# quadjr/aframe-gaussian-splatting

Hardware: AMD Instinct MI355X
Metric: frames/sec @1920x1080 (sort+project+bin+blend per frame, 1M-splat train.splat-shaped scene) (higher is better)
Workload: dtype f32

## Files before the change

aframe-gaussian-splatting_amd/csrc/gs_render.hip:

```cpp
#include "gs_internal.h"
#include "gs_sh.h"

namespace {

#define GS_DPP_ADD(V, CTRL, ROWS) (V) += (uint32_t)__builtin_amdgcn_update_dpp(0, (int)(V), (CTRL), (ROWS), 0xF, false)
__device__ __forceinline__ uint32_t row16_sum(uint32_t v)
{
#ifdef GS_DEBUG_DPP_MAX
    const uint32_t v0_ = v;
#endif
    GS_DPP_ADD(v, 0xB1, 0xF);
    GS_DPP_ADD(v, 0x4E, 0xF);
    GS_DPP_ADD(v, 0x141, 0xF);
    GS_DPP_ADD(v, 0x140, 0xF);
#ifdef GS_DEBUG_DPP_MAX
    { uint32_t c = v0_; for (int m = 8; m >= 1; m >>= 1) c += __shfl_xor(c, m, 16); if (c != v) __builtin_trap(); }
#endif
    return v;
}
__device__ __forceinline__ uint32_t wave_sum(uint32_t v)
{
#ifdef GS_DEBUG_DPP_MAX
    uint32_t c_ = v; for (int m = 32; m >= 1; m >>= 1) c_ += __shfl_xor(c_, m, 64);
#endif
// ... 538 lines not shown
#pragma unroll
        for (uint32_t k = 0; k < 4; k++) {
            s_rrun[4u * l + k] = er; s_rpair[4u * l + k] = ep; if (ITEMS) s_item[4u * l + k] = ei;
            er += rt[k].x; ep += rt[k].y; ei += ni[k];
        }
        if (l == 63) { s_rrun[GS_BLOCK] = er; s_rpair[GS_BLOCK] = ep; if (ITEMS) s_item[GS_BLOCK] = ei; *s_total = sp64; }
    }
    __syncthreads();
    return *s_total;
}

template <int ROUND>
__device__ __forceinline__ void k_row_scan_body(uint32_t *__restrict__ row_cnt, uint2 *__restrict__ row_tot, const GsControl *ctl,
                                                uint32_t near_count, uint32_t rc_stride, uint32_t tiles_y, uint32_t *__restrict__ mask,
                                                uint32_t mask_words)
{
    __shared__ uint32_t s_w[4];
    __shared__ unsigned long long s_p[4];
    uint32_t j_lo, j_hi;
    round_range<ROUND>(ctl, near_count, j_lo, j_hi);
    const uint32_t nch = (j_hi - j_lo + GS_BLOCK - 1) / GS_BLOCK;
    const int lane = threadIdx.x & 63, w = threadIdx.x >> 6;
    const uint32_t per = (nch + GS_BLOCK - 1) / GS_BLOCK;
    const uint32_t lo = min(threadIdx.x * per, nch), hi = min(lo + per, nch);
    for (uint32_t row = blockIdx.x; row < tiles_y; row += gridDim.x) {
        if (ROUND == 0) for (uint32_t i = threadIdx.x; i < mask_words; i += GS_BLOCK) mask[row * mask_words + i] = 0u;
        uint32_t *__restrict__ rc = row_cnt + (size_t)row * rc_stride;
        uint32_t sr = 0;
        unsigned long long sp = 0;
        for (uint32_t c = lo; c < hi; c++) { const uint32_t v = rc[c]; sr += v & 0x1FFu; sp += v >> 9; }
        uint32_t total;
        uint32_t run = block_exscan(sr, s_w, lane, w, total);
        const unsigned long long tp = block_sum64(sp, s_p, lane, w);
        for (uint32_t c = lo; c < hi; c++) { const uint32_t v = rc[c]; rc[c] = run; run += v & 0x1FFu; }
        if (threadIdx.x == 0) row_tot[row] = make_uint2(total, tp > 0xFFFFFFFFull ? 0xFFFFFFFFu : (uint32_t)tp);
    }
}

template <int ROUND>
__global__ __launch_bounds__(GS_BLOCK) void k_row_scan(uint32_t *__restrict__ row_cnt, uint2 *__restrict__ row_tot, const GsControl *ctl,
                                                       uint32_t near_count, uint32_t rc_stride, uint32_t tiles_y, uint32_t *__restrict__ mask,
                                                       uint32_t mask_words)
{
    k_row_scan_body<ROUND>(row_cnt, row_tot, ctl, near_count, rc_stride, tiles_y, mask, mask_words);
}

template <int ROUND>
__device__ __forceinline__ void round_books(GsControl *ctl, unsigned long long I, uint32_t runs, uint32_t j_lo, uint32_t j_hi, uint32_t near_count,
                                            const uint32_t *__restrict__ part_vis, uint32_t nparts, int last_round, uint32_t pair_cap)
{
    __shared__ uint32_t s_vis;
    const uint32_t tid = threadIdx.x;
    const int lane = threadIdx.x & 63;
    if (tid == 0) s_vis = 0;
    __syncthreads();
    uint32_t v = 0;
    if (j_hi > j_lo) for (uint32_t i = tid; i < nparts; i += GS_BLOCK) v += part_vis[i];
#pragma unroll
    for (int m = 32; m >= 1; m >>= 1) v += __shfl_xor(v, m, 64);
    if (lane == 0 && v) atomicAdd(&s_vis, v);
    __syncthreads();
    if (tid == 0) {
        const uint32_t total = I > 0xFFFFFFFFull ? 0xFFFFFFFFu : (uint32_t)I;
        ctl->vis_total = 0; ctl->n_emit_extra = 0;
        ctl->n_runs = (ROUND == 0 ? 0u : ctl->n_runs) + runs;
        if (ROUND == 0) { ctl->n_visible = 0; ctl->n_pairs_frame = 0; ctl->want_frame = 0; }
        else { ctl->unsat_round0 = ctl->unsat_count; if (ctl->unsat_count) ctl->unsat_events += 1; }
        ctl->j_lo = j_lo; ctl->j_hi = j_hi;
        ctl->scan_total = total;
        ctl->want_frame = (ctl->want_frame + total < total) ? 0xFFFFFFFFu : ctl->want_frame + total;
        if (ctl->want_frame > ctl->max_total) ctl->max_total = ctl->want_frame;
        if (total > pair_cap) { ctl->pair_overflow = 1; ctl->overflow_sticky = 1; ctl->n_pairs = 0; }
        else if (ROUND == 0) { ctl->pair_overflow = 0; ctl->n_pairs = total; }
        else ctl->n_pairs = ctl->pair_overflow ? 0u : total;
        ctl->n_visible += s_vis; ctl->n_pairs_frame += ctl->n_pairs;
        if (ROUND == 0 && near_count != 0xFFFFFFFFu) ctl->unsat_count = 0;
        if (last_round) {
            ctl->acc_frames += 1; ctl->acc_sorted += ctl->n_kept; ctl->acc_visible += ctl->n_visible; ctl->acc_pairs += ctl->n_pairs_frame;
        }
    }
    __syncthreads();
}

template <int ROUND>
__device__ __forceinline__ void k_emit_runs_body(const gsm::Projected *__restrict__ proj, const uint2 *__restrict__ rect,
                                                 const uint32_t *__restrict__ tile_count, const uint32_t *__restrict__ row_cnt,
                                                 const uint2 *__restrict__ row_tot, const GsFrameUniforms &u,
                                                 uint32_t *__restrict__ run_geom, uint32_t *__restrict__ run_ref,
                                                 const uint32_t *__restrict__ mask, GsControl *ctl, uint32_t pair_cap, uint2 *__restrict__ row_runs,
                                                 const uint32_t *__restrict__ part_vis, uint32_t nparts, int last_round)
{
    __shared__ float s_rec[GS_BLOCK][6];
    __shared__ uint32_t s_rows[GS_BLOCK], s_t[GS_BLOCK];
    __shared__ unsigned long long s_m[GS_BLOCK][4];
    __shared__ uint32_t s_rowrun[GS_BLOCK + 1], s_rowpair[GS_BLOCK + 1], s_base[GS_BLOCK];
    __shared__ uint32_t s_nbig, s_nmid;
    __shared__ unsigned long long s_p[4];
    const uint32_t tid = threadIdx.x;
    const int lane = threadIdx.x & 63, w = threadIdx.x >> 6;
    const uint32_t tiles_y = (uint32_t)u.tiles_y;
    const unsigned long long I = row_prefixes<false>(row_tot, tiles_y, s_rowrun, s_rowpair, nullptr, s_p);
    uint32_t j_lo, j_hi;
    round_range<ROUND>(ctl, u.near_count, j_lo, j_hi);
    const bool overflow = I > pair_cap || (ROUND == 1 && ctl->pair_overflow);
    if (blockIdx.x == 0) {
        round_books<ROUND>(ctl, I, s_rowrun[GS_BLOCK], j_lo, j_hi, u.near_count, part_vis, nparts, last_round, pair_cap);
        if (ROUND == 0 && tid < tiles_y) row_runs[tid] = make_uint2(s_rowrun[tid], overflow ? 0u : s_rowrun[tid + 1] - s_rowrun[tid]);
    }
    if (overflow) return;
    const uint32_t nchunks = (j_hi - j_lo + GS_BLOCK - 1) / GS_BLOCK;
    for (uint32_t c = blockIdx.x; c < nchunks; c += gridDim.x) {
        s_m[tid][0] = 0ull; s_m[tid][1] = 0ull; s_m[tid][2] = 0ull; s_m[tid][3] = 0ull;
        if (tid == 0) { s_nbig = 0; s_nmid = 0; }
        if (tid < tiles_y) s_base[tid] = s_rowrun[tid] + row_cnt[(size_t)tid * u.rc_stride + c];
        __syncthreads();
        const uint32_t j = j_lo + c * GS_BLOCK + tid;
        const uint32_t cnt = j < j_hi ? tile_count[j] : 0u;
        bool own = false;
        uint32_t ty0 = 0, ty1 = 0;
        gsm::Projected p;
        p.cx = p.cy = p.ax = p.ay = p.bx = p.by = 0.0f;
        uint32_t own_runs = 0, own_present = 0;
        if (cnt) {
            const uint2 rc = rect[j];
            if (rc.x & (1u << 14)) {
                own = true;
                ty0 = rc.x >> 16; ty1 = ty0 + ((rc.x >> 15) & 1u);
                own_runs = rc.y; own_present = (rc.x >> 12) & 3u;
            } else {
                const float4 *src = reinterpret_cast<const float4 *>(proj + j);
                const float4 ra = src[0]; const float2 rb = *reinterpret_cast<const float2 *>(src + 1);
                p.cx = ra.x; p.cy = ra.y; p.ax = ra.z; p.ay = ra.w; p.bx = rb.x; p.by = rb.y;
                ty0 = rc.x >> 16; ty1 = rc.y >> 16;
                const uint32_t q = (ty1 - ty0 >= 16) ? (GS_BLOCK - 1u - atomicAdd(&s_nbig, 1u)) : atomicAdd(&s_nmid, 1u);
                s_rec[q][0] = p.cx; s_rec[q][1] = p.cy; s_rec[q][2] = p.ax; s_rec[q][3] = p.ay; s_rec[q][4] = p.bx; s_rec[q][5] = p.by;
                s_rows[q] = ty0 | (ty1 << 16); s_t[q] = tid;
            }
        }
        __syncthreads();
        const uint32_t nmid = s_nmid, nbig = s_nbig;
#define GS_RUN_ONE(PP, EE, T, TY, FN) do { uint32_t a_, n_;                                                                       \
            gsm::splat_tile_row(PP, EE, (int)(TY), u.H, u.x0, u.x1b, a_, n_);                                                     \
            if (n_ && (ROUND == 0 || mask_count(mask + (TY) * u.mask_words, a_, n_))) { FN((T), (TY), a_, n_); } } while (0)
#define GS_RUN_PASS(FN) do {                                                                                                      \
            if (own) {                                                                                                            \
                for (uint32_t ty = ty0; ty <= ty1; ty++) if ((own_present >> (ty - ty0)) & 1u) {                                  \
                    const uint32_t r_ = own_runs >> (16u * (ty - ty0)), a_ = r_ & 0xFFu, n_ = ((r_ >> 8) & 0xFFu) + 1u;           \
                    if (ROUND == 0 || mask_count(mask + ty * u.mask_words, a_, n_)) { FN(tid, ty, a_, n_); } } }                  \
            for (uint32_t mi = (uint32_t)w * 4u + ((uint32_t)lane >> 4); mi < nmid; mi += 16u) {                                  \
                gsm::Projected q;                                                                                                 \
                q.cx = s_rec[mi][0]; q.cy = s_rec[mi][1]; q.ax = s_rec[mi][2]; q.ay = s_rec[mi][3]; q.bx = s_rec[mi][4]; q.by = s_rec[mi][5]; \
                gsm::EllipseRows e; gsm::ellipse_rows_setup(q, e);                                                                \
                const uint32_t ty = (s_rows[mi] & 0xFFFFu) + ((uint32_t)lane & 15u);                                              \
                if (ty <= (s_rows[mi] >> 16)) GS_RUN_ONE(q, e, s_t[mi], ty, FN); }                                                \
            for (uint32_t bq = (uint32_t)w; bq < nbig; bq += 4u) {                                                                \
                const uint32_t bi = GS_BLOCK - 1u - bq;                                                                           \
                gsm::Projected q;                                                                                                 \
                q.cx = s_rec[bi][0]; q.cy = s_rec[bi][1]; q.ax = s_rec[bi][2]; q.ay = s_rec[bi][3]; q.bx = s_rec[bi][4]; q.by = s_rec[bi][5]; \
                gsm::EllipseRows e; gsm::ellipse_rows_setup(q, e);                                                                \
                for (uint32_t ty = (s_rows[bi] & 0xFFFFu) + (uint32_t)lane; ty <= (s_rows[bi] >> 16); ty += 64u) GS_RUN_ONE(q, e, s_t[bi], ty, FN); } \
        } while (0)
#define GS_RUN_MARK(T, TY, A, N) atomicOr(&s_m[TY][(T) >> 6], 1ull << ((T) & 63u))
        GS_RUN_PASS(GS_RUN_MARK);
        __syncthreads();
#define GS_RUN_WRITE(T, TY, A, N) do { const uint32_t wq_ = (T) >> 6;                                                             \
            uint32_t rank_ = (uint32_t)__popcll(s_m[TY][wq_] & ((1ull << ((T) & 63u)) - 1ull));                                   \
            for (uint32_t k_ = 0; k_ < wq_; k_++) rank_ += (uint32_t)__popcll(s_m[TY][k_]);                                       \
            const uint32_t slot_ = s_base[TY] + rank_;                                                                            \
            run_geom[slot_] = (A) | ((N) << 16); run_ref[slot_] = j_lo + c * GS_BLOCK + (T); } while (0)
        GS_RUN_PASS(GS_RUN_WRITE);
#undef GS_RUN_WRITE
#undef GS_RUN_MARK
#undef GS_RUN_PASS
#undef GS_RUN_ONE
        __syncthreads();
    }
}

template <int ROUND>
__global__ __launch_bounds__(GS_BLOCK) void k_emit_runs(const gsm::Projected *__restrict__ proj, const uint2 *__restrict__ rect,
                                                        const uint32_t *__restrict__ tile_count, const uint32_t *__restrict__ row_cnt,
                                                        const uint2 *__restrict__ row_tot, GsFrameUniforms u,
                                                        uint32_t *__restrict__ run_geom, uint32_t *__restrict__ run_ref,
                                                        const uint32_t *__restrict__ mask, GsControl *ctl, uint32_t pair_cap, uint2 *__restrict__ row_runs,
                                                        const uint32_t *__restrict__ part_vis, uint32_t nparts, int last_round)
{
    k_emit_runs_body<ROUND>(proj, rect, tile_count, row_cnt, row_tot, u, run_geom, run_ref, mask, ctl, pair_cap, row_runs, part_vis, nparts, last_round);
}

template <int ROUND>
__device__ __forceinline__ void k_seg_count_body(const uint32_t *__restrict__ run_geom, const uint2 *__restrict__ row_tot, int *__restrict__ seg_diff,
                                                 const GsFrameUniforms &u, const GsControl *ctl, uint32_t pair_cap)
{
    __shared__ uint32_t s_rrun[GS_BLOCK + 1], s_rpair[GS_BLOCK + 1], s_item[GS_BLOCK + 1];
    __shared__ int s_d[GS_BLOCK + 1];
    __shared__ unsigned long long s_p[4];
    const uint32_t tid = threadIdx.x, tiles_y = (uint32_t)u.tiles_y;
    const unsigned long long I = row_prefixes<true>(row_tot, tiles_y, s_rrun, s_rpair, s_item, s_p);
    if (I > pair_cap || (ROUND == 1 && ctl->pair_overflow)) return;
    const uint32_t NI = s_item[GS_BLOCK];
    for (uint32_t item = blockIdx.x; item < NI; item += gridDim.x) {
        uint32_t row = 0;
#pragma unroll
        for (uint32_t step = GS_BLOCK / 2; step; step >>= 1) { const uint32_t t = row + step; if (t < tiles_y && s_item[t] <= item) row = t; }
        const uint32_t seg = item - s_item[row];
        const uint32_t rb = s_rrun[row], nr = s_rrun[row + 1] - rb;
        const uint32_t S = list_seg_len(nr), s0 = seg * S, s1 = min(nr, s0 + S);
        s_d[tid] = 0;
        if (tid == 0) s_d[GS_BLOCK] = 0;
        __syncthreads();
        for (uint32_t i0 = s0; i0 < s1; i0 += GS_LIST_LOADS * GS_BLOCK) {
            uint32_t g[GS_LIST_LOADS];
#pragma unroll
            for (uint32_t k = 0; k < GS_LIST_LOADS; k++) { const uint32_t i = i0 + k * GS_BLOCK + tid; g[k] = i < s1 ? run_geom[rb + i] : 0u; }
#pragma unroll
            for (uint32_t k = 0; k < GS_LIST_LOADS; k++) {
                const uint32_t i = i0 + k * GS_BLOCK + tid;
                if (i < s1) { const uint32_t t0 = g[k] & 0xFFFFu; atomicAdd(&s_d[t0], 1); atomicSub(&s_d[t0 + (g[k] >> 16)], 1); }
            }
        }
        __syncthreads();
        seg_diff[(size_t)item * GS_BLOCK + tid] = s_d[tid];
        __syncthreads();
    }
}

template <int ROUND>
__global__ __launch_bounds__(GS_BLOCK) void k_seg_count(const uint32_t *__restrict__ run_geom, const uint2 *__restrict__ row_tot, int *__restrict__ seg_diff,
                                                        GsFrameUniforms u, const GsControl *ctl, uint32_t pair_cap)
{
    k_seg_count_body<ROUND>(run_geom, row_tot, seg_diff, u, ctl, pair_cap);
}

__device__ __forceinline__ unsigned long long wave_incl_scan_u64(unsigned long long v, int lane)
{
#pragma unroll
    for (int d = 1; d < 64; d <<= 1) {
        const unsigned long long t = ((unsigned long long)__shfl_up((uint32_t)(v >> 32), d, 64) << 32) | __shfl_up((uint32_t)v, d, 64);
        if (lane >= d) v += t;
    }
    return v;
}

template <int ROUND, bool SEGC>
__device__ __forceinline__ void k_lists_body(const uint32_t *__restrict__ run_geom, const uint32_t *__restrict__ run_ref,
                                             const uint2 *__restrict__ row_tot, const int *__restrict__ seg_diff, uint32_t *__restrict__ lists, uint2 *__restrict__ tile_range,
                                             const GsFrameUniforms &u, const uint32_t *__restrict__ mask, const GsControl *ctl, uint32_t pair_cap)
{
    __shared__ uint32_t s_rrun[GS_BLOCK + 1], s_rpair[GS_BLOCK + 1], s_item[GS_BLOCK + 1];
    __shared__ unsigned long long s_d[GS_BLOCK + 1];
    __shared__ __attribute__((aligned(16))) unsigned long long s_m[GS_BLOCK][4];
    __shared__ uint32_t s_r[GS_BLOCK];
    __shared__ uint32_t s_off[GS_BLOCK], s_on[GS_BLOCK];
    __shared__ uint32_t s_w[4];
    __shared__ unsigned long long s_p[4];
    const uint32_t tid = threadIdx.x;
    const int lane = threadIdx.x & 63, w = threadIdx.x >> 6;
    const uint32_t tiles_x = (uint32_t)u.tiles_x, tiles_y = (uint32_t)u.tiles_y;
    const unsigned long long I = row_prefixes<true>(row_tot, tiles_y, s_rrun, s_rpair, s_item, s_p);
    const uint32_t NI = s_item[GS_BLOCK];
    const bool overflow = I > pair_cap || (ROUND == 1 && ctl->pair_overflow);
    __syncthreads();
    for (uint32_t item = blockIdx.x; item < NI; item += gridDim.x) {
        uint32_t row = 0;
#pragma unroll
        for (uint32_t step = GS_BLOCK / 2; step; step >>= 1) { const uint32_t t = row + step; if (t < tiles_y && s_item[t] <= item) row = t; }
        const uint32_t seg = item - s_item[row];
        const uint32_t rb = s_rrun[row], nr = overflow ? 0u : s_rrun[row + 1] - rb, pb = s_rpair[row];
        const uint32_t S = list_seg_len(nr), s0 = seg * S, s1 = min(nr, s0 + S);
        if (SEGC) {
// ... 169 lines not shown
    }
    return m;
}

template <bool COUNT, int ROUND, bool SCENE, bool SUB, bool WALK = false, bool SURF = false>
__device__ __forceinline__ void k_blend_body(const uint2 *__restrict__ tile_range, const void *__restrict__ pairs,
                                             const gsm::Projected *__restrict__ proj, const GsFrameUniforms &u,
                                             uint8_t *__restrict__ out, float4 *__restrict__ state, uint32_t *__restrict__ mask,
                                             const float *__restrict__ zwin, const float *__restrict__ scene_depth,
                                             const uint32_t *__restrict__ scene_rgba, GsControl *ctl,
                                             const uint32_t *__restrict__ sorted = nullptr)
{
    __shared__ float4 s_ent[3 * (GS_BLEND_BATCH + 1)];
    __shared__ float s_z[GS_BLEND_BATCH + 2];
    __shared__ __attribute__((aligned(16))) uint8_t s_list[SUB ? GS_SUBTILE_GROUPS * GS_SUBTILE_STRIDE : 16];
    __shared__ uint32_t s_j[SURF ? 2 * GS_BLEND_BATCH : WALK ? GS_BLEND_BATCH : 1];
    static_assert(!WALK || (!COUNT && ROUND == 0 && !SUB), "the row walk serves round 0 of plain frames");
    static_assert(!SURF || (!COUNT && !SUB && !WALK), "a surface frame takes the tile lists");
    const int lane = threadIdx.x;
    if (blockIdx.x == 0 && lane == 0 && u.status && ctl->pair_overflow) atomicOr(u.status, 2u);
    if (ROUND == 1 && ctl->j_hi == 0) return;
    static_assert(GS_BLEND_BATCH == 64, "the sub-tile lists name a batch's entries by the lane that staged them");
    if (SUB && lane == 0) {
        if (SCENE) s_z[GS_SUBTILE_INERT] = 0.0f;
        s_ent[3 * GS_SUBTILE_INERT] = make_float4(-1.0e9f, -1.0e9f, 1.0f, 1.0f); s_ent[3 * GS_SUBTILE_INERT + 1] = make_float4(1.0f, 1.0f, 0.0f, 0.0f);
        s_ent[3 * GS_SUBTILE_INERT + 2] = make_float4(0.0f, 0.0f, 0.0f, 0.0f);
    }
    const uint32_t ntiles = (uint32_t)u.tiles_x * (uint32_t)u.tiles_y;
    const bool span = u.rc_stride != 0u;
    for (uint32_t tile = blockIdx.x; tile < ntiles; tile += gridDim.x) {
    const uint32_t tx = tile % (uint32_t)u.tiles_x, ty = tile / (uint32_t)u.tiles_x;
    if (ROUND == 1 && !((mask[ty * u.mask_words + (tx >> 5)] >> (tx & 31)) & 1u)) continue;
    const int xb = u.x0 + (int)tx * GS_TILE + (lane & 3) * 4;
    const int r = (int)ty * GS_TILE + (lane >> 2);
    const bool row_in = r < u.H;
    const float fy = (float)(u.H - 1 - r) + 0.5f;
    const bool no_early = (COUNT && !(u.flags & GS_RENDER_COUNT_EVALUATED)) || (u.flags & GS_RENDER_NO_EARLY_OUT);
    const float t_eps = no_early ? -1.0f : u.t_eps;
    f2 fxA = { (float)xb + 0.5f, (float)(xb + 1) + 0.5f }, fxB = { (float)(xb + 2) + 0.5f, (float)(xb + 3) + 0.5f };
    const f2 qmA = { (row_in && xb < u.x1b) ? 4.0f : -1.0f, (row_in && xb + 1 < u.x1b) ? 4.0f : -1.0f };
    const f2 qmB = { (row_in && xb + 2 < u.x1b) ? 4.0f : -1.0f, (row_in && xb + 3 < u.x1b) ? 4.0f : -1.0f };
    f2 TA = { qmA.x > 0.0f ? 1.0f : 0.0f, qmA.y > 0.0f ? 1.0f : 0.0f }, TB = { qmB.x > 0.0f ? 1.0f : 0.0f, qmB.y > 0.0f ? 1.0f : 0.0f };
    const f2 cwA = { qmA.x > 0.0f ? GS_BLEND_W_C_IN : GS_BLEND_W_C_OUT, qmA.y > 0.0f ? GS_BLEND_W_C_IN : GS_BLEND_W_C_OUT };
    const f2 cwB = { qmB.x > 0.0f ? GS_BLEND_W_C_IN : GS_BLEND_W_C_OUT, qmB.y > 0.0f ? GS_BLEND_W_C_IN : GS_BLEND_W_C_OUT };
    f2 crA = { 0, 0 }, crB = { 0, 0 }, cgA = { 0, 0 }, cgB = { 0, 0 }, cbA = { 0, 0 }, cbB = { 0, 0 };
    float zb0 = 3.0e38f, zb1 = 3.0e38f, zb2 = 3.0e38f, zb3 = 3.0e38f;
    if (SCENE && u.has_depth && row_in) {
        const float *zr = scene_depth + (size_t)r * u.W + xb;
        if (xb < u.x1b) zb0 = zr[0];
        if (xb + 1 < u.x1b) zb1 = zr[1];
        if (xb + 2 < u.x1b) zb2 = zr[2];
        if (xb + 3 < u.x1b) zb3 = zr[3];
    }
    float4 *st = state + ((size_t)tile * 64 + lane) * 4;
    if (ROUND == 1) {
        const float4 t = st[0], c0 = st[1], c1 = st[2], c2 = st[3];
        TA = (f2){ t.x, t.y }; TB = (f2){ t.z, t.w };
        crA = (f2){ c0.x, c0.y }; crB = (f2){ c0.z, c0.w }; cgA = (f2){ c1.x, c1.y }; cgB = (f2){ c1.z, c1.w };
        cbA = (f2){ c2.x, c2.y }; cbB = (f2){ c2.z, c2.w };
    }
#define GS_LANE_LIVE() (fmaxf(fmaxf(TA.x, TA.y), fmaxf(TB.x, TB.y)) >= t_eps)
    f2 kbig = { GS_BLEND_W_K, GS_BLEND_W_K }, kone = { 1.0f, 1.0f };
    if (GS_BLEND_FACTOR == 2 && !COUNT && !SCENE && !SURF) {
        kbig = -kbig;
        asm volatile("" : "+v"(kbig));
    } else asm volatile("" : "+v"(kbig), "+v"(kone));
    bool live = GS_LANE_LIVE();
    uint32_t nfr = 0, staged = 0, evaluated = 0;
    uint32_t sfj0 = 0xFFFFFFFFu, sfj1 = 0xFFFFFFFFu, sfj2 = 0xFFFFFFFFu, sfj3 = 0xFFFFFFFFu;
    float sfz0 = 1.0f, sfz1 = 1.0f, sfz2 = 1.0f, sfz3 = 1.0f;
    uint32_t sfc0 = 0xFFFFFFFFu, sfc1 = 0xFFFFFFFFu, sfc2 = 0xFFFFFFFFu, sfc3 = 0xFFFFFFFFu;
    const uint2 range = WALK ? tile_range[ty] : tile_range[tile];
    if (!WALK && u.split_min && range.y - range.x >= u.split_min) continue;
    const uint32_t *__restrict__ run_geom = reinterpret_cast<const uint32_t *>(pairs), *__restrict__ run_ref = run_geom + u.walk_ref;
    uint32_t cur = range.x + range.y;
    uint32_t j_mine = 0xFFFFFFFFu, nb_last = 0, e_l = 0;
    const uint32_t need_known = ctl->need_near[tile % GS_NEED_WORDS];

    for (uint32_t end = range.y; WALK ? cur > range.x : end > range.x;) {
        uint32_t nb;
        if (WALK) {
            nb = 0;
            do {
                const uint32_t avail = cur - range.x;
                bool hit = false;
                uint32_t jr = 0;
                if ((uint32_t)lane < avail) {
                    const uint32_t i = cur - 1u - (uint32_t)lane, g = run_geom[i];
                    jr = run_ref[i];
                    hit = tx - (g & 0xFFFFu) < (g >> 16);
                }
                const unsigned long long bal = __ballot(hit);
                const uint32_t pos = nb + __builtin_amdgcn_mbcnt_hi((uint32_t)(bal >> 32), __builtin_amdgcn_mbcnt_lo((uint32_t)bal, 0u));
                if (hit && pos < GS_BLEND_BATCH) s_j[pos] = jr;
                const uint32_t nh = (uint32_t)__popcll(bal);
                if (nb + nh > GS_BLEND_BATCH) {
                    const unsigned long long last = __ballot(hit && pos == GS_BLEND_BATCH - 1u);
                    cur -= (uint32_t)__ffsll((long long)last);
                    nb = GS_BLEND_BATCH;
                } else {
                    nb += nh;
                    cur -= min(avail, 64u);
                }
            } while (nb < GS_BLEND_BATCH && cur > range.x);
            if (nb == 0) break;
            __syncthreads();
        } else nb = min((uint32_t)GS_BLEND_BATCH, end - range.x);
        staged += nb;
        nb_last = nb; e_l = 0;
        uint32_t m16 = 0;
        const bool sfo0 = SURF && TA.x >= 0.5f, sfo1 = SURF && TA.y >= 0.5f, sfo2 = SURF && TB.x >= 0.5f, sfo3 = SURF && TB.y >= 0.5f;
#pragma unroll
        for (int h = 0; h < GS_BLEND_BATCH / 64; h++) {
            const uint32_t slot = h * 64 + lane;
            if (slot < nb) {
                const uint32_t j = WALK ? s_j[slot] : span ? reinterpret_cast<const uint32_t *>(pairs)[end - 1 - slot] : reinterpret_cast<const uint2 *>(pairs)[end - 1 - slot].y;
                const float4 *src = reinterpret_cast<const float4 *>(proj + j);
                const float4 ra = src[0], rb = src[1];
                if (GS_BLEND_BATCH == 64) j_mine = j;
                if (SUB) m16 = subtile_mask(ra, rb.x, rb.y, (float)(u.x0 + (int)tx * GS_TILE), (int)ty * GS_TILE, u.H);
                s_ent[3 * slot] = make_float4(ra.x, ra.y, ra.z, rb.x);
                s_ent[3 * slot + 1] = make_float4(ra.w, rb.y, 0.0f, 0.0f);
                const uint32_t rgba = __float_as_uint(rb.z);
                const float a255 = rb.w * (1.0f / 255.0f);
                s_ent[3 * slot + 2] = make_float4(-rb.w, (float)(rgba & 0xFF) * a255, (float)((rgba >> 8) & 0xFF) * a255, (float)((rgba >> 16) & 0xFF) * a255);
                if (SCENE) s_z[slot] = u.has_depth ? zwin[j] : 0.0f;
                if (SURF) { s_j[slot] = j; s_j[GS_BLEND_BATCH + slot] = __float_as_uint(zwin[j]); }
            }
        }
        if (lane == 0 && (nb & 1)) {
            if (SCENE) s_z[nb] = 0.0f;
            s_ent[3 * nb] = make_float4(-1.0e9f, -1.0e9f, 1.0f, 1.0f);
            s_ent[3 * nb + 1] = make_float4(1.0f, 1.0f, 0.0f, 0.0f);
            s_ent[3 * nb + 2] = make_float4(0.0f, 0.0f, 0.0f, 0.0f);
        }
        __syncthreads();
        uint32_t cnt_max = nb;
        bool split = false;
        if (SUB && nb >= 8u) {
            uint32_t cm = 0;
            uint32_t *lw = reinterpret_cast<uint32_t *>(s_list);
            for (uint32_t i = (uint32_t)lane; i < GS_SUBTILE_GROUPS * GS_SUBTILE_STRIDE / 4u; i += 64u) lw[i] = GS_SUBTILE_INERT * 0x01010101u;
#pragma unroll
            for (int g = 0; g < GS_SUBTILE_GROUPS; g++) {
                const unsigned long long bal = __ballot((m16 >> g) & 1u);
                const uint32_t c = (uint32_t)__popcll(bal);
                cm = c > cm ? c : cm;
                const uint32_t pos = __builtin_amdgcn_mbcnt_hi((uint32_t)(bal >> 32), __builtin_amdgcn_mbcnt_lo((uint32_t)bal, 0u));
                if ((m16 >> g) & 1u) s_list[g * GS_SUBTILE_STRIDE + pos] = (uint8_t)lane;
            }
            split = cm * 16u <= nb * GS_SUBTILE_KEEP_NUM;
            if (split) {
                cnt_max = cm;
                __syncthreads();
            }
        }
#define GS_BLEND_Q(K, EB, qA, qB)                                                                                      \
                const float4 a_##K = *reinterpret_cast<const float4 *>(EB); const f2 ab_##K = *reinterpret_cast<const f2 *>((EB) + 16); \
                const f2 axbx_##K = { a_##K.z, a_##K.w };                                                               \
                const f2 dyab_##K = (f2)(fy - a_##K.y) * ab_##K;                               \
                const f2 dxA_##K = fxA - a_##K.x, dxB_##K = fxB - a_##K.x;                                              \
                const f2 pxA_##K = fma2_lo12(dxA_##K, axbx_##K, dyab_##K), pxB_##K = fma2_lo12(dxB_##K, axbx_##K, dyab_##K); \
                const f2 pyA_##K = fma2_hi12(dxA_##K, axbx_##K, dyab_##K), pyB_##K = fma2_hi12(dxB_##K, axbx_##K, dyab_##K); \
                const f2 qA = fma2(pxA_##K, pxA_##K, pyA_##K * pyA_##K), qB = fma2(pxB_##K, pxB_##K, pyB_##K * pyB_##K);
#define GS_BLEND_APPLY(qA, qB, EB, zz, ss)                                                                             \
                {                                                                                                      \
                    bool p0 = qA.x <= qmA.x, p1 = qA.y <= qmA.y, p2 = qB.x <= qmB.x, p3 = qB.y <= qmB.y;               \
                    if (SCENE) { p0 = p0 && zz <= zb0; p1 = p1 && zz <= zb1; p2 = p2 && zz <= zb2; p3 = p3 && zz <= zb3; } \
                    if (live & (p0 | p1 | p2 | p3)) {                                  \
                              \
                        const float2 cl_ = *reinterpret_cast<const float2 *>((EB) + 32);                               \
                        const float2 ch_ = *reinterpret_cast<const float2 *>((EB) + 40);                               \
                        const float nalpha = cl_.x;                                            \
                                       \
                           \
                        const f2 tA = qA * (f2)(-1.44269502f), tB = qB * (f2)(-1.44269502f);                            \
                        const f2 EA = { p0 ? __builtin_amdgcn_exp2f(tA.x) : 0.0f, p1 ? __builtin_amdgcn_exp2f(tA.y) : 0.0f }; \
                        const f2 EB_ = { p2 ? __builtin_amdgcn_exp2f(tB.x) : 0.0f, p3 ? __builtin_amdgcn_exp2f(tB.y) : 0.0f }; \
                         \
                        const f2 eA = EA * TA, eB = EB_ * TB;                                                          \
                        TA = fma2((f2)(nalpha), eA, TA); TB = fma2((f2)(nalpha), eB, TB);                              \
                        crA = fma2((f2)(cl_.y), eA, crA); crB = fma2((f2)(cl_.y), eB, crB);                            \
                        cgA = fma2((f2)(ch_.x), eA, cgA); cgB = fma2((f2)(ch_.x), eB, cgB);                            \
                                      \
                        const f2 chv_ = { ch_.x, ch_.y };                                                              \
                        cbA = fma2_hi0(chv_, eA, cbA); cbB = fma2_hi0(chv_, eB, cbB);                                  \
                        if (COUNT) nfr += (uint32_t)p0 + (uint32_t)p1 + (uint32_t)p2 + (uint32_t)p3;                   \
                        if (SURF) {                                           \
                            const uint32_t s_ = (ss);                                                                  \
                            sfc0 = TA.x < 0.5f ? min(sfc0, s_) : sfc0; sfc1 = TA.y < 0.5f ? min(sfc1, s_) : sfc1;      \
                            sfc2 = TB.x < 0.5f ? min(sfc2, s_) : sfc2; sfc3 = TB.y < 0.5f ? min(sfc3, s_) : sfc3;      \
                        }                                                                                              \
                        live = GS_LANE_LIVE();                                                                         \
                    }                                                                                                  \
                }
#if GS_BLEND_FACTOR == 2
#define GS_BLEND_W(qA, qB) const f2 wA = fma2_clamp(qA, kbig, cwA), wB = fma2_clamp(qB, kbig, cwB);
#else
#define GS_BLEND_W(qA, qB) const f2 wA = fma2_clamp(qmA - qA, kbig, kone), wB = fma2_clamp(qmB - qB, kbig, kone);
// ... 312 lines not shown
                        E[k + 1] = p1 ? __expf(-q.y) : 0.0f;
                    }
#pragma unroll
                    for (uint32_t k = 0; k < GS_PX_GROUP; k++) {
                        const float e = E[k] * T;
                        T = fmaf(cc[k].y, e, T);
                        cr = fmaf(cc[k].x, e, cr); cg = fmaf(cc[k].z, e, cg); cb = fmaf(cc[k].w, e, cb);
                    }
                    live = T >= t_eps;
                    e_l = min(s4 + (GS_PX_GROUP - 1u), nb - 1u);
                    if (!live) break;
                }
            }
            end -= nb;
            GS_WAVE_LDS_SYNC();
            if (__all(!live)) break;
        }
        const bool wave_live = __any(live);
        if (lane == 0) s_live[w] = wave_live ? 1u : 0u;
        if (!(u.flags & GS_RENDER_NO_EARLY_OUT)) {
            const bool more = ROUND == 0 && u.near_count < ctl->n_kept;
            if (!wave_live || !more) {
                uint32_t e_max = e_l;
#pragma unroll
                for (int m = 32; m >= 1; m >>= 1) e_max = max(e_max, (uint32_t)__shfl_xor((int)e_max, m, 64));
                if (lane == 0) {
                    const uint32_t V = ctl->n_kept;
                    uint32_t need = 0xFFFFFFFFu;
                    if (!wave_live) {
                        need = 0u;
                        if (range.y > range.x && end_w > range.x + e_max) {
                            const uint32_t li = end_w - 1u - e_max;
                            const uint32_t jf = span ? reinterpret_cast<const uint32_t *>(pairs)[li] : reinterpret_cast<const uint2 *>(pairs)[li].y;
                            need = jf < V ? V - jf : 0u;
                        }
                    }
                    if (need > need_known) atomicMax(&ctl->need_near[tile % GS_NEED_WORDS], need);
                }
            }
        }
        __syncthreads();
        const bool tile_live = (s_live[0] | s_live[1] | s_live[2] | s_live[3]) != 0u;
        if (ROUND == 0 && u.near_count < ctl->n_kept && tile_live) {
            st[0] = T; st[4] = cr; st[8] = cg; st[12] = cb;
            if (threadIdx.x == 0) {
                atomicOr(&mask[ty * u.mask_words + (tx >> 5)], 1u << (tx & 31)); atomicAdd(&ctl->unsat_count, 1u);
                if (u.skip_round1) { ctl->round1_missed = 1; if (u.status) atomicOr(u.status, 1u); }
            }
        }
        if (in) {
            float b0 = u.bg[0], b1 = u.bg[1], b2 = u.bg[2], b3 = u.bg[3];
            if (SCENE && u.has_scene_rgba) {
                const uint32_t c = scene_rgba[(size_t)r * u.W + px];
                b0 = (float)(c & 0xFF) / 255.0f; b1 = (float)((c >> 8) & 0xFF) / 255.0f;
                b2 = (float)((c >> 16) & 0xFF) / 255.0f; b3 = (float)(c >> 24) / 255.0f;
            }
            const float o0 = fmaf(T, b0, cr), o1 = fmaf(T, b1, cg), o2 = fmaf(T, b2, cb), o3 = fmaf(T, b3, 1.0f - T);
            const int sw = u.out_pitch;
            const int orow = (u.flags & GS_RENDER_FLIP_Y) ? (u.H - 1 - r) : r;
            reinterpret_cast<uint32_t *>(out)[(size_t)orow * sw + (px - u.x0)] =
                (uint32_t)(fminf(fmaxf(o0, 0.0f), 1.0f) * 255.0f + 0.5f) | ((uint32_t)(fminf(fmaxf(o1, 0.0f), 1.0f) * 255.0f + 0.5f) << 8) |
                ((uint32_t)(fminf(fmaxf(o2, 0.0f), 1.0f) * 255.0f + 0.5f) << 16) | ((uint32_t)(fminf(fmaxf(o3, 0.0f), 1.0f) * 255.0f + 0.5f) << 24);
        }
        __syncthreads();
    }
#undef GS_PX_FETCH
#undef GS_WAVE_LDS_SYNC
}

template <int ROUND, bool SCENE>
__global__ __launch_bounds__(256) void k_blend_px(const uint2 *__restrict__ tile_range, const void *__restrict__ pairs,
                                                  const gsm::Projected *__restrict__ proj, GsFrameUniforms u,
                                                  uint8_t *__restrict__ out, float4 *__restrict__ state, uint32_t *__restrict__ mask,
                                                  const float *__restrict__ zwin, const float *__restrict__ scene_depth,
                                                  const uint32_t *__restrict__ scene_rgba, GsControl *ctl)
{
    k_blend_px_body<ROUND, SCENE>(tile_range, pairs, proj, u, out, state, mask, zwin, scene_depth, scene_rgba, ctl);
}

int bits_for(uint32_t n) { int b = 1; while (b < 32 && (1u << b) < n) b++; return b; }

template <int ROUND, bool RUNS, bool SH, bool AA, bool HL> GS_BODY(F_project, (k_project<ROUND, RUNS, SH, AA, HL>), (k_project_body<ROUND, RUNS, SH, AA, HL>));
template <int ROUND> GS_BODY(F_row_scan, (k_row_scan<ROUND>), (k_row_scan_body<ROUND>));
template <int ROUND> GS_BODY(F_emit_runs, (k_emit_runs<ROUND>), (k_emit_runs_body<ROUND>));
template <int ROUND> GS_BODY(F_seg_count, (k_seg_count<ROUND>), (k_seg_count_body<ROUND>));
template <int ROUND, bool SEGC> GS_BODY(F_lists, (k_lists<ROUND, SEGC>), (k_lists_body<ROUND, SEGC>));
template <int ROUND> GS_BODY(F_pairs_check, (k_pairs_check<ROUND>), (k_pairs_check_body<ROUND>));
template <int ROUND> GS_BODY(F_emit, (k_emit<ROUND>), (k_emit_body<ROUND>));
GS_BODY(F_tile_ranges, (k_tile_ranges), (k_tile_ranges_body));
template <int ROUND, bool SCENE, bool SUB, bool WALK> GS_BODY(F_blend, (k_blend<false, ROUND, SCENE, SUB, WALK>), (k_blend_body<false, ROUND, SCENE, SUB, WALK>));
template <int ROUND, bool SCENE> GS_BODY(F_blend_px, (k_blend_px<ROUND, SCENE>), (k_blend_px_body<ROUND, SCENE>));
template <int ROUND, bool SCENE, bool SUB> GS_BODY(F_blend_count, (k_blend<true, ROUND, SCENE, SUB>), (k_blend_body<true, ROUND, SCENE, SUB>));
template <int ROUND, bool SCENE> GS_BODY(F_blend_surf, (k_blend_surf<ROUND, SCENE>), (k_blend_body<false, ROUND, SCENE, false, false, true>));


template <int ROUND, int NF>
int launch_blend(gs_ctx *const S[], const GsFrameUniforms V[], uint8_t *const out[], const void *const lists[])
{
    gs_ctx *ctx = S[0];
    const GsFrameUniforms &u = V[0];
    const uint32_t ntiles = (uint32_t)u.tiles_x * (uint32_t)u.tiles_y;
    hipStream_t st = ctx->stream;
    const uint32_t gb = ROUND == 1 ? (ntiles < 1024 ? ntiles : 1024) : ntiles;
    const bool scene = u.has_depth || u.has_scene_rgba;
    const bool count = (u.flags & GS_RENDER_COUNT_FRAGS) != 0;
    if (NF != 1 && (count || u.record_staged || u.surface)) { snprintf(GS_ERRBUF(ctx), GS_ERRLEN, "paired blend: a measurement or surface frame"); return GS_E_STATE; }
    GsFrameUniforms W[NF];
    for (int k = 0; k < NF; k++) W[k] = V[k];
    if (count || u.record_staged) W[0].split_min = 0;
    const bool walk = ROUND == 0 && u.row_walk;
    const auto args = [&](int k) {
        return gs_pack_make(walk ? (const uint2 *)S[k]->row_tot + GS_BLOCK : (const uint2 *)S[k]->tile_range, lists[k], (const gsm::Projected *)S[k]->proj, W[k], out[k],
                            S[k]->state, S[k]->unsat_mask, (const float *)S[k]->zwin, (const float *)S[k]->scene_depth, (const uint32_t *)S[k]->scene_rgba, S[k]->ctl);
    };
    if constexpr (NF == 1) {
        if (u.surface) {
            const auto sargs = [&](int) {
                return gs_pack_make((const uint2 *)ctx->tile_range, lists[0], (const gsm::Projected *)ctx->proj, W[0], out[0], ctx->state, ctx->unsat_mask, (const float *)ctx->zwin,
                                    (const float *)ctx->scene_depth, (const uint32_t *)ctx->scene_rgba, ctx->ctl, (const uint32_t *)ctx->sorted);
            };
            gs_flag(scene, [&](auto SC) { gs_launch<1, F_blend_surf<ROUND, decltype(SC)::value>, 64>(gb, st, 0, sargs); });
            GS_HIP(hipGetLastError());
            return GS_OK;
        }
    }
    if (walk) {
        gs_flag(scene, [&](auto SC) { gs_launch<NF, F_blend<ROUND, decltype(SC)::value, false, ROUND == 0>, 64>(gb, st, 0, args); });
        GS_HIP(hipGetLastError());
        return GS_OK;
    }
    if (W[0].split_min) gs_flag(scene, [&](auto SC) { gs_launch<NF, F_blend_px<ROUND, decltype(SC)::value>, 256>(ntiles < 2048 ? ntiles : 2048, st, 0, args); });
    gs_flag(scene, [&](auto SC) { gs_flag(u.subtile != 0, [&](auto SB) {
        if constexpr (NF == 1) { if (count) { gs_launch<1, F_blend_count<ROUND, decltype(SC)::value, decltype(SB)::value>, 64>(gb, st, 0, args); return; } }
        gs_launch<NF, F_blend<ROUND, decltype(SC)::value, decltype(SB)::value, false>, 64>(gb, st, 0, args);
    }); });
    GS_HIP(hipGetLastError());
    return GS_OK;
}

#define GS_ROWCNT_MAX ((size_t)1 << 25)
uint32_t span_list_stride(const gs_ctx *ctx, const GsFrameUniforms &u, uint32_t jrange)
{
    const gs_ctx *P = gs_root(const_cast<gs_ctx *>(ctx));
    if (P->bin_mode == 1) return 0;
    if (u.tiles_x > GS_BLOCK || u.tiles_y > GS_BLOCK) return 0;
    const uint32_t stride = gs_div_up(jrange, GS_BLOCK) + 1u;
    if ((size_t)stride * (size_t)u.tiles_y > GS_ROWCNT_MAX) return 0;
    return stride;
}

size_t gs_row_table_entries(size_t n, uint32_t tiles_y)
{
    const size_t e = (size_t)(gs_div_up(n, GS_BLOCK) + 1u) * (size_t)tiles_y;
    return e > GS_ROWCNT_MAX ? 0 : e;
}

int gs_ensure_row_tables(gs_ctx *ctx, size_t entries)
{
    if (entries <= ctx->row_cnt_cap && ctx->row_tot && ctx->seg_diff) return GS_OK;
    GS_HIP(hipStreamSynchronize(ctx->stream));
    if (entries > ctx->row_cnt_cap) {
        if (ctx->row_cnt) (void)hipFree(ctx->row_cnt);
        ctx->row_cnt = nullptr; ctx->row_cnt_cap = 0;
        const size_t cap = entries + entries / 4;
        GS_HIP(hipMalloc((void **)&ctx->row_cnt, cap * sizeof(uint32_t)));
        ctx->row_cnt_cap = cap;
    }
    if (!ctx->row_tot) { GS_HIP(hipMalloc((void **)&ctx->row_tot, 2 * GS_BLOCK * sizeof(uint2))); ctx->row_tot_cap = 2 * GS_BLOCK; }
    if (!ctx->seg_diff) GS_HIP(hipMalloc((void **)&ctx->seg_diff, (size_t)GS_BLOCK * (GS_LIST_SEGS + 1u) * GS_BLOCK * sizeof(int)));
    return GS_OK;
}

template <int ROUND>
bool row_walk_round(const GsFrameUniforms &u)
{
    return ROUND == 0 && u.row_walk && !(u.flags & GS_RENDER_COUNT_FRAGS) && !u.record_staged && !u.subtile && !u.split_min;
}

template <int ROUND, bool RUNS, int NF>
void launch_project(gs_ctx *const S[], const GsFrameUniforms F[], uint32_t g)
{
    hipStream_t st = S[0]->stream;
    const auto args = [&](int k) {
        return gs_pack_make((const uint32_t *)S[k]->sorted, (const uint4 *)S[k]->splat, F[k], S[k]->proj, S[k]->rect, S[k]->tile_count, RUNS ? S[k]->row_cnt : S[k]->spine,
                            S[k]->part_vis, (const uint32_t *)S[k]->unsat_mask, S[k]->zwin, S[k]->ctl);
    };
    gs_flag(F[0].sh_degree != 0, [&](auto SH) { gs_flag(F[0].antialias != 0, [&](auto AA) { gs_flag(F[0].highlight != 0, [&](auto HL) {
        gs_launch<NF, F_project<ROUND, RUNS, decltype(SH)::value, decltype(AA)::value, decltype(HL)::value>, GS_BLOCK>(g, st, 0, args);
    }); }); });
}

template <int ROUND, int NF>
int run_round_spans(gs_ctx *const S[], const GsFrameUniforms U[], uint8_t *const out[], bool last_round, uint32_t g, uint32_t stride)
{
    gs_ctx *ctx = S[0];
    const GsFrameUniforms &u = U[0];
    hipStream_t st = ctx->stream;
    for (int k = 0; k < NF; k++) { const int rcc = gs_ensure_row_tables(S[k], (size_t)stride * (size_t)u.tiles_y); if (rcc != GS_OK) return rcc; }
    GsFrameUniforms V[NF];
    uint32_t *geom[NF], *ref[NF], *lists[NF];
    for (int k = 0; k < NF; k++) {
        V[k] = U[k];
        V[k].rc_stride = stride;
        V[k].row_walk = row_walk_round<ROUND>(u) ? 1u : 0u;
        V[k].walk_ref = (uint32_t)S[k]->pair_cap;
        geom[k] = reinterpret_cast<uint32_t *>(S[k]->pair_a); ref[k] = geom[k] + S[k]->pair_cap; lists[k] = reinterpret_cast<uint32_t *>(S[k]->pair_b);
    }
    launch_project<ROUND, true, NF>(S, V, g);
    GS_HIP(hipGetLastError());
    if (ROUND == 0) GS_PROF_RECORD(ctx, 3);
    gs_launch<NF, F_row_scan<ROUND>, GS_BLOCK>((uint32_t)u.tiles_y, st, 0, [&](int k) {
        return gs_pack_make(S[k]->row_cnt, S[k]->row_tot, (const GsControl *)S[k]->ctl, U[k].near_count, stride, (uint32_t)u.tiles_y, S[k]->unsat_mask, u.mask_words); });
    gs_launch<NF, F_emit_runs<ROUND>, GS_BLOCK>(g, st, 0, [&](int k) {
        return gs_pack_make((const gsm::Projected *)S[k]->proj, (const uint2 *)S[k]->rect, (const uint32_t *)S[k]->tile_count, (const uint32_t *)S[k]->row_cnt,
                            (const uint2 *)S[k]->row_tot, V[k], geom[k], ref[k], (const uint32_t *)S[k]->unsat_mask, S[k]->ctl, (uint32_t)S[k]->pair_cap,
                            S[k]->row_tot + GS_BLOCK, (const uint32_t *)S[k]->part_vis, g, last_round ? 1 : 0); });
    const void *fpairs[NF];
    if (V[0].row_walk) {
        GS_HIP(hipGetLastError());
        if (ROUND == 0) GS_PROF_RECORD(ctx, 4);
        for (int k = 0; k < NF; k++) fpairs[k] = geom[k];
        return launch_blend<ROUND, NF>(S, V, out, fpairs);
    }
    uint32_t gl = (uint32_t)u.tiles_y * GS_LIST_SEGS; if (gl > (ROUND == 1 ? 512u : 2048u)) gl = ROUND == 1 ? 512u : 2048u;
    const int segc_opt = gs_root(ctx)->seg_count_opt;
    const bool segc = ROUND == 0 && segc_opt != 0 &&
                      (segc_opt == 2 || __atomic_load_n(&gs_root(ctx)->run_hint, __ATOMIC_RELAXED) > GS_SEGC_RUNS_PER_ROW * (uint32_t)u.tiles_y);
    if (segc) for (int k = 0; k < NF; k++) S[k]->stats.seg_count = 1u;
    if (segc)
        gs_launch<NF, F_seg_count<ROUND>, GS_BLOCK>(gl, st, 0, [&](int k) {
            return gs_pack_make((const uint32_t *)geom[k], (const uint2 *)S[k]->row_tot, S[k]->seg_diff, V[k], (const GsControl *)S[k]->ctl, (uint32_t)S[k]->pair_cap); });
    gs_flag(segc, [&](auto SEGC) {
        gs_launch<NF, F_lists<ROUND, decltype(SEGC)::value>, GS_BLOCK>(gl, st, 0, [&](int k) {
            return gs_pack_make((const uint32_t *)geom[k], (const uint32_t *)ref[k], (const uint2 *)S[k]->row_tot, (const int *)S[k]->seg_diff, lists[k], S[k]->tile_range, V[k],
                                (const uint32_t *)S[k]->unsat_mask, (const GsControl *)S[k]->ctl, (uint32_t)S[k]->pair_cap); }); });
    GS_HIP(hipGetLastError());
    if (ROUND == 0) GS_PROF_RECORD(ctx, 4);
    for (int k = 0; k < NF; k++) fpairs[k] = lists[k];
    return launch_blend<ROUND, NF>(S, V, out, fpairs);
}

template <int ROUND, int NF>
int run_round(gs_ctx *const S[], const GsFrameUniforms U[], uint8_t *const out[], bool last_round)
{
    gs_ctx *ctx = S[0];
    const GsFrameUniforms &u = U[0];
    const uint32_t ntiles = (uint32_t)u.tiles_x * (uint32_t)u.tiles_y;
    const uint32_t Vmax = (uint32_t)ctx->n;
    hipStream_t st = ctx->stream;
    uint32_t g = gs_div_up(Vmax, GS_BLOCK); if (g > GS_MAX_PART) g = GS_MAX_PART;
    const uint32_t small = 512;
    if (ROUND == 1 && g > small) g = small;
    if (ROUND == 0 && u.near_count != 0xFFFFFFFFu) { const uint32_t gn = gs_div_up(u.near_count < Vmax ? u.near_count : Vmax, GS_BLOCK); if (gn < g) g = gn ? gn : 1; }
    uint32_t pc = (uint32_t)S[0]->pair_cap;
    for (int k = 1; k < NF; k++) if ((uint32_t)S[k]->pair_cap < pc) pc = (uint32_t)S[k]->pair_cap;
    const uint32_t ph = ROUND == 1 ? (uint32_t)(small * GS_CHUNK_S) : __atomic_load_n(&gs_root(ctx)->pair_hint, __ATOMIC_RELAXED);
    const uint32_t jrange = ROUND == 0 ? (u.near_count != 0xFFFFFFFFu && u.near_count < Vmax ? u.near_count : Vmax) : Vmax;
    if (const uint32_t stride = span_list_stride(ctx, u, jrange)) return run_round_spans<ROUND, NF>(S, U, out, last_round, g, stride);
    const int tb = bits_for(ntiles);
    GsFrameUniforms V[NF];
    for (int k = 0; k < NF; k++) { V[k] = U[k]; V[k].rc_stride = 0; V[k].row_walk = 0; }
    launch_project<ROUND, false, NF>(S, U, g);
    GS_HIP(hipGetLastError());
    if (ROUND == 0) GS_PROF_RECORD(ctx, 3);
    gs_launch<NF, F_pairs_check<ROUND>, GS_BLOCK>(1, st, 0, [&](int k) {
        return gs_pack_make(S[k]->ctl, (uint32_t)S[k]->pair_cap, S[k]->spine, (const uint32_t *)S[k]->part_vis, g, U[k].near_count, last_round ? 1 : 0, S[k]->unsat_mask,
                            (uint32_t)u.tiles_y * u.mask_words, S[k]->emit_extra); });
    uint32_t ge = g + (ROUND == 1 ? 0u : gs_div_up(ph ? ph : pc, GS_EMIT_PAIRS)); if (ge > GS_MAX_PART) ge = GS_MAX_PART;
    gs_launch<NF, F_emit<ROUND>, GS_BLOCK>(ge, st, 0, [&](int k) {
        return gs_pack_make((const gsm::Projected *)S[k]->proj, (const uint2 *)S[k]->rect, (const uint32_t *)S[k]->tile_count, (const uint32_t *)S[k]->spine,
                            (const uint2 *)S[k]->emit_extra, V[k], S[k]->pair_a, (const uint32_t *)S[k]->unsat_mask, (const GsControl *)S[k]->ctl); });
    GS_HIP(hipGetLastError());
    GsRadixIO io[NF];
    const void *fpairs[NF];
    const int b1 = tb <= 9 ? tb : (tb + 1) / 2, b2 = tb - b1;
    for (int k = 0; k < NF; k++) { io[k] = GsRadixIO{ S[k]->pair_a, S[k]->pair_b, &S[k]->ctl->n_pairs, nullptr, nullptr }; fpairs[k] = S[k]->pair_b; }
    int rc = gs_radix_pass<NF>(S, io, GS_RADIX_PACKED, GS_RADIX_PACKED, pc, ph, 0, b1);
    if (rc != GS_OK) return rc;
    if (b2) {
        for (int k = 0; k < NF; k++) { io[k].in = S[k]->pair_b; io[k].out = S[k]->pair_a; fpairs[k] = S[k]->pair_a; }
        rc = gs_radix_pass<NF>(S, io, GS_RADIX_PACKED, GS_RADIX_PACKED, pc, ph, b1, b2);
        if (rc != GS_OK) return rc;
    }
    gs_launch<NF, F_tile_ranges, GS_BLOCK>(ROUND == 1 ? small : 2048, st, 0, [&](int k) {
        return gs_pack_make((const uint2 *)fpairs[k], S[k]->tile_range, ntiles, ROUND, (const GsControl *)S[k]->ctl); });
    GS_HIP(hipGetLastError());
    if (ROUND == 0) GS_PROF_RECORD(ctx, 4);
    return launch_blend<ROUND, NF>(S, V, out, fpairs);
}

}

int gs_row_tables_ensure(gs_ctx *ctx, size_t entries) { return gs_ensure_row_tables(ctx, entries); }
size_t gs_row_tables_entries(size_t n, uint32_t tiles_y) { return gs_row_table_entries(n, tiles_y); }

uint32_t gs_round0_binning(const gs_ctx *L, const GsFrameUniforms &u)
{
    const uint32_t Vmax = (uint32_t)L->n;
    const uint32_t jrange = u.near_count != 0xFFFFFFFFu && u.near_count < Vmax ? u.near_count : Vmax;
// ... 76 lines not shown
```

Baseline: 21070.

## Pack row-walk run geometry into 16-bit entries and scan two per lane

When the row walk is active in round 0, the run emitter now stores each run's start column and length-minus-one as 8-bit fields in a 16-bit entry instead of a 32-bit word. The blend walk reads one 32-bit word per lane that covers two runs, tests both, and gathers run_ref only for hits through stored slot indices. This halves the bytes scanned per tile row and doubles the runs examined per wave iteration, aiming to cut the cost of the walk loop. In exchange it assumes column and length fit in 8 bits, adds an indirection on run_ref in the gather, and makes the batch-boundary bookkeeping more involved.

```diff
diff --git a/aframe-gaussian-splatting_amd/csrc/gs_render.hip b/aframe-gaussian-splatting_amd/csrc/gs_render.hip
--- a/aframe-gaussian-splatting_amd/csrc/gs_render.hip
+++ b/aframe-gaussian-splatting_amd/csrc/gs_render.hip
@@ -644,7 +644,7 @@
     __syncthreads();
 }
 
-template <int ROUND>
+template <int ROUND, bool W16 = false>
 __device__ __forceinline__ void k_emit_runs_body(const gsm::Projected *__restrict__ proj, const uint2 *__restrict__ rect,
                                                  const uint32_t *__restrict__ tile_count, const uint32_t *__restrict__ row_cnt,
                                                  const uint2 *__restrict__ row_tot, const GsFrameUniforms &u,
@@ -729,7 +729,9 @@
             uint32_t rank_ = (uint32_t)__popcll(s_m[TY][wq_] & ((1ull << ((T) & 63u)) - 1ull));                                   \
             for (uint32_t k_ = 0; k_ < wq_; k_++) rank_ += (uint32_t)__popcll(s_m[TY][k_]);                                       \
             const uint32_t slot_ = s_base[TY] + rank_;                                                                            \
-            run_geom[slot_] = (A) | ((N) << 16); run_ref[slot_] = j_lo + c * GS_BLOCK + (T); } while (0)
+            if (W16) reinterpret_cast<uint16_t *>(run_geom)[slot_] = (uint16_t)((A) | (((N) - 1u) << 8));                          \
+            else run_geom[slot_] = (A) | ((N) << 16);                                                                             \
+            run_ref[slot_] = j_lo + c * GS_BLOCK + (T); } while (0)
         GS_RUN_PASS(GS_RUN_WRITE);
 #undef GS_RUN_WRITE
 #undef GS_RUN_MARK
@@ -739,7 +741,7 @@
     }
 }
 
-template <int ROUND>
+template <int ROUND, bool W16 = false>
 __global__ __launch_bounds__(GS_BLOCK) void k_emit_runs(const gsm::Projected *__restrict__ proj, const uint2 *__restrict__ rect,
                                                         const uint32_t *__restrict__ tile_count, const uint32_t *__restrict__ row_cnt,
                                                         const uint2 *__restrict__ row_tot, GsFrameUniforms u,
@@ -747,7 +749,8 @@
                                                         const uint32_t *__restrict__ mask, GsControl *ctl, uint32_t pair_cap, uint2 *__restrict__ row_runs,
                                                         const uint32_t *__restrict__ part_vis, uint32_t nparts, int last_round)
 {
-    k_emit_runs_body<ROUND>(proj, rect, tile_count, row_cnt, row_tot, u, run_geom, run_ref, mask, ctl, pair_cap, row_runs, part_vis, nparts, last_round);
+    static_assert(!W16 || ROUND == 0, "the row walk serves round 0");
+    k_emit_runs_body<ROUND, W16>(proj, rect, tile_count, row_cnt, row_tot, u, run_geom, run_ref, mask, ctl, pair_cap, row_runs, part_vis, nparts, last_round);
 }
 
 template <int ROUND>
@@ -1083,25 +1086,25 @@
         if (WALK) {
             nb = 0;
             do {
-                const uint32_t avail = cur - range.x;
-                bool hit = false;
-                uint32_t jr = 0;
-                if ((uint32_t)lane < avail) {
-                    const uint32_t i = cur - 1u - (uint32_t)lane, g = run_geom[i];
-                    jr = run_ref[i];
-                    hit = tx - (g & 0xFFFFu) < (g >> 16);
-                }
-                const unsigned long long bal = __ballot(hit);
-                const uint32_t pos = nb + __builtin_amdgcn_mbcnt_hi((uint32_t)(bal >> 32), __builtin_amdgcn_mbcnt_lo((uint32_t)bal, 0u));
-                if (hit && pos < GS_BLEND_BATCH) s_j[pos] = jr;
-                const uint32_t nh = (uint32_t)__popcll(bal);
+                const uint32_t D = (cur - 1u) >> 1, d = D - (uint32_t)lane, left = cur - range.x;
+                const bool in = (uint32_t)lane <= D;
+                const uint32_t g = run_geom[in ? d : 0u], i0 = 2u * d, i1 = i0 + 1u;
+                const bool hit1 = in && i1 - range.x < left && tx - ((g >> 16) & 0xFFu) <= (g >> 24);
+                const bool hit0 = in && i0 - range.x < left && tx - (g & 0xFFu) <= ((g >> 8) & 0xFFu);
+                const unsigned long long bal1 = __ballot(hit1), bal0 = __ballot(hit0);
+                const uint32_t pos1 = __builtin_amdgcn_mbcnt_hi((uint32_t)(bal0 >> 32), __builtin_amdgcn_mbcnt_lo((uint32_t)bal0,
+                                      __builtin_amdgcn_mbcnt_hi((uint32_t)(bal1 >> 32), __builtin_amdgcn_mbcnt_lo((uint32_t)bal1, nb))));
+                const uint32_t pos0 = pos1 + (hit1 ? 1u : 0u);
+                if (hit1 && pos1 < GS_BLEND_BATCH) s_j[pos1] = i1;
+                if (hit0 && pos0 < GS_BLEND_BATCH) s_j[pos0] = i0;
+                const uint32_t nh = (uint32_t)__popcll(bal1) + (uint32_t)__popcll(bal0);
                 if (nb + nh > GS_BLEND_BATCH) {
-                    const unsigned long long last = __ballot(hit && pos == GS_BLEND_BATCH - 1u);
-                    cur -= (uint32_t)__ffsll((long long)last);
+                    const unsigned long long last1 = __ballot(hit1 && pos1 == GS_BLEND_BATCH - 1u), last0 = __ballot(hit0 && pos0 == GS_BLEND_BATCH - 1u);
+                    cur = last1 ? 2u * (D + 1u - (uint32_t)__ffsll((long long)last1)) + 1u : 2u * (D + 1u - (uint32_t)__ffsll((long long)last0));
                     nb = GS_BLEND_BATCH;
                 } else {
                     nb += nh;
-                    cur -= min(avail, 64u);
+                    cur = D >= 63u && 2u * (D - 63u) > range.x ? 2u * (D - 63u) : range.x;
                 }
             } while (nb < GS_BLEND_BATCH && cur > range.x);
             if (nb == 0) break;
@@ -1115,7 +1118,7 @@
         for (int h = 0; h < GS_BLEND_BATCH / 64; h++) {
             const uint32_t slot = h * 64 + lane;
             if (slot < nb) {
-                const uint32_t j = WALK ? s_j[slot] : span ? reinterpret_cast<const uint32_t *>(pairs)[end - 1 - slot] : reinterpret_cast<const uint2 *>(pairs)[end - 1 - slot].y;
+                const uint32_t j = WALK ? run_ref[s_j[slot]] : span ? reinterpret_cast<const uint32_t *>(pairs)[end - 1 - slot] : reinterpret_cast<const uint2 *>(pairs)[end - 1 - slot].y;
                 const float4 *src = reinterpret_cast<const float4 *>(proj + j);
                 const float4 ra = src[0], rb = src[1];
                 if (GS_BLEND_BATCH == 64) j_mine = j;
@@ -1594,7 +1597,7 @@
 
 template <int ROUND, bool RUNS, bool SH, bool AA, bool HL> GS_BODY(F_project, (k_project<ROUND, RUNS, SH, AA, HL>), (k_project_body<ROUND, RUNS, SH, AA, HL>));
 template <int ROUND> GS_BODY(F_row_scan, (k_row_scan<ROUND>), (k_row_scan_body<ROUND>));
-template <int ROUND> GS_BODY(F_emit_runs, (k_emit_runs<ROUND>), (k_emit_runs_body<ROUND>));
+template <int ROUND, bool W16> GS_BODY(F_emit_runs, (k_emit_runs<ROUND, W16>), (k_emit_runs_body<ROUND, W16>));
 template <int ROUND> GS_BODY(F_seg_count, (k_seg_count<ROUND>), (k_seg_count_body<ROUND>));
 template <int ROUND, bool SEGC> GS_BODY(F_lists, (k_lists<ROUND, SEGC>), (k_lists_body<ROUND, SEGC>));
 template <int ROUND> GS_BODY(F_pairs_check, (k_pairs_check<ROUND>), (k_pairs_check_body<ROUND>));
@@ -1723,10 +1726,11 @@
     if (ROUND == 0) GS_PROF_RECORD(ctx, 3);
     gs_launch<NF, F_row_scan<ROUND>, GS_BLOCK>((uint32_t)u.tiles_y, st, 0, [&](int k) {
         return gs_pack_make(S[k]->row_cnt, S[k]->row_tot, (const GsControl *)S[k]->ctl, U[k].near_count, stride, (uint32_t)u.tiles_y, S[k]->unsat_mask, u.mask_words); });
-    gs_launch<NF, F_emit_runs<ROUND>, GS_BLOCK>(g, st, 0, [&](int k) {
-        return gs_pack_make((const gsm::Projected *)S[k]->proj, (const uint2 *)S[k]->rect, (const uint32_t *)S[k]->tile_count, (const uint32_t *)S[k]->row_cnt,
-                            (const uint2 *)S[k]->row_tot, V[k], geom[k], ref[k], (const uint32_t *)S[k]->unsat_mask, S[k]->ctl, (uint32_t)S[k]->pair_cap,
-                            S[k]->row_tot + GS_BLOCK, (const uint32_t *)S[k]->part_vis, g, last_round ? 1 : 0); });
+    gs_flag(ROUND == 0 && V[0].row_walk, [&](auto W16) {
+        gs_launch<NF, F_emit_runs<ROUND, ROUND == 0 && decltype(W16)::value>, GS_BLOCK>(g, st, 0, [&](int k) {
+            return gs_pack_make((const gsm::Projected *)S[k]->proj, (const uint2 *)S[k]->rect, (const uint32_t *)S[k]->tile_count, (const uint32_t *)S[k]->row_cnt,
+                                (const uint2 *)S[k]->row_tot, V[k], geom[k], ref[k], (const uint32_t *)S[k]->unsat_mask, S[k]->ctl, (uint32_t)S[k]->pair_cap,
+                                S[k]->row_tot + GS_BLOCK, (const uint32_t *)S[k]->part_vis, g, last_round ? 1 : 0); }); });
     const void *fpairs[NF];
     if (V[0].row_walk) {
         GS_HIP(hipGetLastError());
```

Measured after the change: 21540, median of 6. 1.02x the previous value.
